# Liz490/multimodal_alzheimer

Measured on AMD Instinct MI355X. Metric: volumes/sec fwd+bwd, 3D-ResNet-10 @128^3 bf16, 1/2/4/8 MI355X; % HBM roofline, higher is better.
Workload: dtype bf16; 1 GPU; BASELINE config 2: Anat_CNN ResNet-10 MRI-only, 1x128^3, batch 8/GPU, weighted CE, Adam, fwd+bwd+step; global_batch=8, parallelism=dp1, step_launch=hip graph replay

## Files before the change

multimodal_alzheimer_amd/csrc/common.h:

```cpp
#pragma once
#include <hip/hip_runtime.h>
#include <stdint.h>

#include "../../include/mmad.h"

typedef float f32x4 __attribute__((ext_vector_type(4)));
typedef __bf16 bf16x8 __attribute__((ext_vector_type(8)));
typedef __bf16 bf16x4 __attribute__((ext_vector_type(4)));
typedef unsigned short u16;
typedef unsigned short u16x8 __attribute__((ext_vector_type(8)));
typedef unsigned short u16x4 __attribute__((ext_vector_type(4)));
typedef uint32_t u32x4 __attribute__((ext_vector_type(4)));

#define LDS_AS __attribute__((address_space(3)))

template <int N>
__device__ __forceinline__ void wait_vm_lgkm0() {
  static_assert(N >= 0 && N <= 63, "vmcnt immediate (6 bits)");
  asm volatile("s_waitcnt vmcnt(%0) lgkmcnt(0)" ::"i"(N) : "memory");
}

__device__ __forceinline__ void raw_barrier() {
  __builtin_amdgcn_s_barrier();
  asm volatile("" ::: "memory");
}

__device__ __forceinline__ void glds16_asm(const void* gsrc, uint32_t lds_addr) {
  uint32_t keep;
  asm volatile(
      "s_mov_b32 %0, m0\n\ts_mov_b32 m0, %2\n\ts_nop 0\n\t"
      "global_load_lds_dwordx4 %1, off\n\ts_mov_b32 m0, %0"
      : "=&s"(keep)
      : "v"(gsrc), "s"(lds_addr)
      : "memory");
}
__device__ __forceinline__ void buf_lds16_asm(uint32_t voff, __amdgpu_buffer_rsrc_t rsrc,
                                              uint32_t lds_addr) {
  uint32_t keep;
  asm volatile(
      "s_mov_b32 %0, m0\n\ts_mov_b32 m0, %3\n\ts_nop 0\n\t"
      "buffer_load_dwordx4 %1, %2, 0 offen lds\n\ts_mov_b32 m0, %0"
      : "=&s"(keep)
      : "v"(voff), "s"(rsrc), "s"(lds_addr)
      : "memory");
}
__device__ __forceinline__ uint32_t lds_addr_of(const void* p) {
  return __builtin_amdgcn_readfirstlane((uint32_t)(uintptr_t)(const LDS_AS void*)p);
}

__device__ __forceinline__ float bf2f(u16 v) { return __uint_as_float(((uint32_t)v) << 16); }
typedef float f32x2 __attribute__((ext_vector_type(2)));
typedef __bf16 bf16x2 __attribute__((ext_vector_type(2)));
__device__ __forceinline__ uint32_t pack_bf16x2(float a, float b) {
  return __builtin_bit_cast(uint32_t, __builtin_convertvector((f32x2){a, b}, bf16x2));
}
__device__ __forceinline__ u16 f2bf(float f) { return (u16)(pack_bf16x2(f, 0.f) & 0xffffu); }

template <typename T> struct Elt;
template <> struct Elt<float> {
  static __device__ __forceinline__ float ld(const float* p, int64_t i) { return p[i]; }
  static __device__ __forceinline__ void st(float* p, int64_t i, float v) { p[i] = v; }
  static constexpr int VEC = 4;
};
template <> struct Elt<u16> {
  static __device__ __forceinline__ float ld(const u16* p, int64_t i) { return bf2f(p[i]); }
  static __device__ __forceinline__ void st(u16* p, int64_t i, float v) { p[i] = f2bf(v); }
  static constexpr int VEC = 8;
};

template <typename T> struct Chunk;
template <> struct Chunk<float> {
  static constexpr int N = 4;
  static __device__ __forceinline__ void load(const float* p, float* v) {
    f32x4 c = *reinterpret_cast<const f32x4*>(p);
    v[0] = c[0]; v[1] = c[1]; v[2] = c[2]; v[3] = c[3];
  }
  static __device__ __forceinline__ void store(float* p, const float* v) {
    f32x4 c; c[0] = v[0]; c[1] = v[1]; c[2] = v[2]; c[3] = v[3];
    *reinterpret_cast<f32x4*>(p) = c;
  }
};
template <> struct Chunk<u16> {
  static constexpr int N = 8;
  static __device__ __forceinline__ void load(const u16* p, float* v) {
    u16x8 c = *reinterpret_cast<const u16x8*>(p);
#pragma unroll
    for (int i = 0; i < 8; ++i) v[i] = bf2f(c[i]);
  }
  static __device__ __forceinline__ void store(u16* p, const float* v) {
    u32x4 c;
#pragma unroll
    for (int i = 0; i < 4; ++i) c[i] = pack_bf16x2(v[2 * i], v[2 * i + 1]);
    *reinterpret_cast<u32x4*>(p) = c;
  }
};

__device__ __forceinline__ u32x4 epi_res_relu(u32x4 v, const u16* res, int relu) {
  float f[8];
  Chunk<u16>::load(reinterpret_cast<const u16*>(&v), f);
  if (res != nullptr) {
    float r[8];
    Chunk<u16>::load(res, r);
#pragma unroll
    for (int e = 0; e < 8; ++e) f[e] += r[e];
  }
  if (relu) {
#pragma unroll
    for (int e = 0; e < 8; ++e) f[e] = fmaxf(f[e], 0.f);
  }
  u32x4 o;
  Chunk<u16>::store(reinterpret_cast<u16*>(&o), f);
  return o;
}

__device__ __forceinline__ float bn_affine(float y, float scale, float shift) {
  return __builtin_fmaf(y, scale, shift);
}
template <typename T>
__device__ __forceinline__ float as_stored(float v) {
  if constexpr (sizeof(T) == 2) return bf2f(f2bf(v));
  else return v;
}

__device__ __forceinline__ float wave_sum(float v) {
#pragma unroll
  for (int o = 32; o > 0; o >>= 1) v += __shfl_xor(v, o, 64);
  return v;
}
__device__ __forceinline__ double wave_sum_d(double v) {
#pragma unroll
  for (int o = 32; o > 0; o >>= 1) v += __shfl_xor(v, o, 64);
  return v;
}

__device__ __forceinline__ uint64_t mix64(uint64_t z) {
  z += 0x9E3779B97F4A7C15ull;
  z = (z ^ (z >> 30)) * 0xBF58476D1CE4E5B9ull;
  z = (z ^ (z >> 27)) * 0x94D049BB133111EBull;
  return z ^ (z >> 31);
}

static inline int hip_status(hipError_t e) { return e == hipSuccess ? MMAD_OK : MMAD_EHIP + (int)e; }
static inline int launch_status() { return hip_status(hipGetLastError()); }
static inline hipStream_t as_stream(void* s) { return reinterpret_cast<hipStream_t>(s); }
static inline int64_t cdiv(int64_t a, int64_t b) { return (a + b - 1) / b; }

__global__ void zero_fill_kernel(uint32_t* __restrict__ p, int64_t words);
int zero_fill(void* p, int64_t bytes, hipStream_t st);
static inline bool is_pow2(int64_t v) { return v > 0 && (v & (v - 1)) == 0; }
static inline int ilog2(int64_t v) { int r = 0; while ((int64_t(1) << r) < v) ++r; return r; }
```

multimodal_alzheimer_amd/csrc/lattice8.hip:

```cpp
#include <atomic>
#include <cstdlib>
#include <type_traits>

#include "bnsum.h"
#include "common.h"
#include "patchconv.h"

namespace {

constexpr int S8 = 8;
constexpr int NC = 8;
constexpr int PL8 = S8 * S8 * NC;
constexpr int RB8 = 64;
constexpr int KC8 = RB8 / 2;
constexpr int PLANE8 = PL8 * RB8;
constexpr int BN8 = 64;
constexpr int BTAP8 = BN8 * RB8;
constexpr int TPS8 = 9;
constexpr int BSLOT8 = TPS8 * BTAP8;
constexpr int NSL8 = 2;
constexpr int NPL8 = 2;
constexpr int RING8 = NPL8 * PLANE8;
constexpr int ZERO8 = RING8 + NSL8 * BSLOT8;
constexpr int MAIN8 = ZERO8 + RB8;
constexpr int CROW8 = BN8 * 2 + 16;
constexpr int EPI8 = PL8 * CROW8 + 7 * 2 * BN8 * 4;
constexpr int LDS8 = MAIN8 > EPI8 ? MAIN8 : EPI8;
constexpr int NT8 = 512;

struct L8 {
  int nb, Cs, Nd, Kpad, nbn, nchunk;
  const u16* res;
  int relu;
  int D, H, W, nz;
  const u16* bny;
  const float *bnsc, *bnsh, *bnmu, *bnis;
  float* bnparts;
};

__device__ __forceinline__ int swz8(int row) { return 3 * ((row >> 3) & 1); }

template <int TN, int NFR>
struct Fr8 {
  bf16x8 b[TN];
  bf16x8 a[NFR];
};

template <int WM, int KY, int WR>
__device__ constexpr bool row_ok(int f) {
  return WR * WM + (f >> 2) + KY >= 0 && WR * WM + (f >> 2) + KY < S8;
}

template <int TN, int WM, int KY, int KX, int WR>
__device__ __forceinline__ void read8(const char* bsl, const char* pl, const uint32_t (&ao)[2],
                                      const char* zp, bool lhi, Fr8<TN, 4 * WR>& f) {
#pragma unroll
  for (int j = 0; j < TN; ++j)
    f.b[j] = *reinterpret_cast<const bf16x8*>(bsl + (KX + 1) * BTAP8 + j * 16 * RB8);
#pragma unroll
  for (int q = 0; q < 4 * WR; ++q) {
    if (row_ok<WM, KY, WR>(q)) {
      constexpr int dummy = 0;
      const int ty = WR * WM + (q >> 2) + KY + dummy, x0 = 2 * (q & 3) + KX;
      const int base = (ty * S8 + x0) * NC * RB8;
      const char* p = pl + base + ao[KX & 1];
      if (KX == -1 && (q & 3) == 0) p = lhi ? p : zp;
      if (KX == 1 && (q & 3) == 3) p = lhi ? zp : p;
      f.a[q] = *reinterpret_cast<const bf16x8*>(p);
    }
  }
}

template <int TN, int WM, int KY, int WR>
__device__ __forceinline__ void mma8(f32x4 (&acc)[4 * WR][TN], const Fr8<TN, 4 * WR>& f) {
#pragma unroll
  for (int q = 0; q < 4 * WR; ++q)
    if (row_ok<WM, KY, WR>(q)) {
#pragma unroll
      for (int j = 0; j < TN; ++j)
        acc[q][j] = __builtin_amdgcn_mfma_f32_16x16x32_bf16(f.a[q], f.b[j], acc[q][j], 0, 0, 0);
    }
}

template <int TN, int WM, int KY, int WR>
__device__ __forceinline__ void stage8(f32x4 (&acc)[4 * WR][TN], const char* bsl,
                                       const char* pl, const uint32_t (&ao)[2], const char* zp,
                                       bool lhi) {
  Fr8<TN, 4 * WR> f0, f1;
  read8<TN, WM, KY, -1, WR>(bsl, pl, ao, zp, lhi, f0);
  read8<TN, WM, KY, 0, WR>(bsl, pl, ao, zp, lhi, f1);
  mma8<TN, WM, KY, WR>(acc, f0);
  read8<TN, WM, KY, 1, WR>(bsl, pl, ao, zp, lhi, f0);
  mma8<TN, WM, KY, WR>(acc, f1);
  mma8<TN, WM, KY, WR>(acc, f0);
}

template <int TN, bool RAG, int WR>
__global__ __launch_bounds__(NT8) void lattice8_conv_kernel(L8 g, const u16* __restrict__ src,
                                                            const u16* __restrict__ wgt,
                                                            const float* __restrict__ bias,
                                                            u16* __restrict__ dst,
                                                            float* __restrict__ stats) {
  extern __shared__ __attribute__((aligned(16))) char smem[];
  char* ring = smem + RING8;
  const int tid = threadIdx.x, lane = tid & 63;
  const int wave = __builtin_amdgcn_readfirstlane(tid >> 6);
  const int nwg = gridDim.x, bid = blockIdx.x;
  const int xcd = bid & 7, qq = nwg >> 3, rr = nwg & 7;
  const int tile = (xcd < rr ? xcd * (qq + 1) : rr * (qq + 1) + (xcd - rr) * qq) + (bid >> 3);
  const int nt = tile % g.nbn;
  const int t2 = tile / g.nbn;
  const int NZ = RAG ? g.nz : S8;
  const int tz = t2 % NZ, n = t2 / NZ;
  constexpr int NFR = 4 * WR;
  constexpr int NWM = 8 / WR, NWN = WR;
  constexpr int BW = 16 * TN * NWN;
  const int n0 = nt * BW;
  constexpr int E = 2 * S8;

  if (tid < RB8 / 16)
    *reinterpret_cast<u32x4*>(smem + ZERO8 + tid * 16) = u32x4{0u, 0u, 0u, 0u};

  const int lrow = lane >> 2;
  int rzk[4];
  uint32_t pofs[4];
#pragma unroll
  for (int k = 0; k < 4; ++k) {
    const int row = (wave * 4 + k) * 16 + lrow;
    const int pos = row >> 3, c = row & 7;
    const int ty = pos >> 3, tx = pos & 7;
    const int pch = (lane & 3) ^ swz8(row);
    if constexpr (RAG) {
      const int y = ((c >> 1) & 1) + 2 * ty, x = (c & 1) + 2 * tx;
      pofs[k] = (uint32_t)((((c >> 2) * g.H + y) * g.W + x) * g.Cs + pch * 8) * 2u;
      rzk[k] = (y < g.H && x < g.W) ? (c >> 2) : -(1 << 20);
    } else {
      const int v = ((c >> 2) * E + ((c >> 1) & 1) + 2 * ty) * E + (c & 1) + 2 * tx;
      pofs[k] = (uint32_t)(v * g.Cs + pch * 8) * 2u;
      rzk[k] = 0;
    }
  }
  const int64_t svox = RAG ? (int64_t)g.D * g.H * g.W : (int64_t)E * E * E;
  const __amdgpu_buffer_rsrc_t rsx = __builtin_amdgcn_make_buffer_rsrc(
      (void*)(src + (int64_t)n * svox * g.Cs), 0,
      (int)__builtin_amdgcn_readfirstlane((uint32_t)(svox * g.Cs * 2)), 0x00020000);
  auto issue_plane_at = [&](int p, int zr, int cc) {
    char* pb = smem + p * PLANE8;
    if constexpr (RAG) {
      constexpr uint32_t OOB = 0x80000000u;
      const int zp = 2 * (tz - 1 + zr);
      const uint32_t zoff = (uint32_t)(zp * g.H * g.W * g.Cs + cc * KC8) * 2u;
#pragma unroll
      for (int k = 0; k < 4; ++k) {
        const bool ok = rzk[k] >= 0 && rzk[k] + zp >= 0 && rzk[k] + zp < g.D;
        buf_lds16_asm(ok ? pofs[k] + zoff : OOB, rsx, lds_addr_of(pb + (wave * 4 + k) * 1024));
      }
    } else {
      const uint32_t zoff = (uint32_t)(2 * (tz - 1 + zr) * E * E * g.Cs + cc * KC8) * 2u;
#pragma unroll
      for (int k = 0; k < 4; ++k) {
        uint32_t o = pofs[k];
        asm volatile("" : "+v"(o));
        buf_lds16_asm(o + zoff, rsx, lds_addr_of(pb + (wave * 4 + k) * 1024));
      }
    }
  };
  constexpr int QB = BW / 16;
  constexpr int NQ9 = 9 * BW / 16, WI9 = (NQ9 + 7) / 8;
  const __amdgpu_buffer_rsrc_t rsw = __builtin_amdgcn_make_buffer_rsrc(
      (void*)wgt, 0, (int)__builtin_amdgcn_readfirstlane((uint32_t)(g.Nd * g.Kpad * 2)),
      0x00020000);
  uint32_t wofs9[WI9];
#pragma unroll
  for (int h = 0; h < WI9; ++h) {
    const int q = min(wave + 8 * h, NQ9 - 1);
    const int row = (q % QB) * 16 + lrow;
    wofs9[h] = (uint32_t)((n0 + row) * g.Kpad + ((lane & 3) ^ swz8(row)) * 8 + (q / QB) * g.Cs) *
               2u;
  }
  auto issue_b9 = [&](int cc, int t0, int sl) {
    const uint32_t so = (uint32_t)(t0 * g.Cs + cc * KC8) * 2u;
#pragma unroll
    for (int h = 0; h < WI9; ++h) {
      const int q = min(wave + 8 * h, NQ9 - 1);
      uint32_t o = wofs9[h];
      asm volatile("" : "+v"(o));
      buf_lds16_asm(o + so, rsw, lds_addr_of(ring + sl * BSLOT8 + (q / QB) * BTAP8 + (q % QB) * 1024));
    }
  };
  const int kz0 = tz == 0 ? 0 : -1, kz1 = tz == NZ - 1 ? 0 : 1;
  const int nkz = kz1 - kz0 + 1;
  const int wm = wave % NWM, wn = wave / NWM;
  const int lr = lane & 15, lk = lane >> 4;
  const bool lhi = (lr >> 3) != 0;
  uint32_t ao[2];
  ao[0] = lr * RB8 + ((lk ^ swz8(lr)) << 4);
  ao[1] = lr * RB8 + ((lk ^ (3 - swz8(lr))) << 4);
  const char* zp = smem + ZERO8 + (lk << 4);
  const uint32_t b_lane = (wn * 16 * TN + lr) * RB8 + ((lk ^ swz8(lr)) << 4);
  f32x4 acc[NFR][TN];
#pragma unroll
  for (int i = 0; i < NFR; ++i)
#pragma unroll
    for (int j = 0; j < TN; ++j) acc[i][j] = f32x4{0.f, 0.f, 0.f, 0.f};

  auto run9 = [&](auto wmc) {
    constexpr int WM = decltype(wmc)::value;
    const int n9 = g.nchunk * nkz;
    issue_plane_at(0, kz0 + 1, 0);
    issue_b9(0, (kz0 + 1) * 9, 0);
    int e = 0;
    for (int c = 0; c < g.nchunk; ++c)
      for (int kzi = 0; kzi < nkz; ++kzi, ++e) {
        wait_vm_lgkm0<0>();
        raw_barrier();
        if (e + 1 < n9) {
          const int c1 = kzi + 1 < nkz ? c : c + 1, kz1 = kz0 + (kzi + 1 < nkz ? kzi + 1 : 0);
          issue_plane_at((e + 1) & 1, kz1 + 1, c1);
          issue_b9(c1, (kz1 + 1) * 9, (e + 1) & 1);
        }
        const char* pl = smem + (e & 1) * PLANE8;
        const char* bs = ring + (e & 1) * BSLOT8 + b_lane;
        stage8<TN, WM, -1, WR>(acc, bs, pl, ao, zp, lhi);
        stage8<TN, WM, 0, WR>(acc, bs + 3 * BTAP8, pl, ao, zp, lhi);
        stage8<TN, WM, 1, WR>(acc, bs + 6 * BTAP8, pl, ao, zp, lhi);
      }
  };
  auto dispatch = [&](auto wmc) {
    if constexpr (decltype(wmc)::value < NWM) run9(wmc);
  };
  switch (wm) {
    case 0: dispatch(std::integral_constant<int, 0>{}); break;
    case 1: dispatch(std::integral_constant<int, 1>{}); break;
    case 2: dispatch(std::integral_constant<int, 2>{}); break;
    case 3: dispatch(std::integral_constant<int, 3>{}); break;
    case 4: dispatch(std::integral_constant<int, 4>{}); break;
    case 5: dispatch(std::integral_constant<int, 5>{}); break;
    case 6: dispatch(std::integral_constant<int, 6>{}); break;
    default: dispatch(std::integral_constant<int, 7>{}); break;
  }
  __syncthreads();

  auto dst_vox = [&](int row) -> int64_t {
    const int pos = row >> 3, c = row & 7;
    const int ty = pos >> 3, tx = pos & 7;
    if constexpr (RAG) {
      const int z = (c >> 2) + 2 * tz, y = ((c >> 1) & 1) + 2 * ty, x = (c & 1) + 2 * tx;
      if (z >= g.D || y >= g.H || x >= g.W) return -1;
      return (((int64_t)n * g.D + z) * g.H + y) * g.W + x;
    }
    return (((int64_t)n * E + (c >> 2) + 2 * tz) * E + ((c >> 1) & 1) + 2 * ty) * E + (c & 1) +
           2 * tx;
  };
  u16* ctile = reinterpret_cast<u16*>(smem);
  uint32_t vmask = 0xffffffffu;
  if constexpr (RAG) {
    vmask = 0;
#pragma unroll 1
    for (int b = 0; b < 4 * NFR; ++b) {
      const int q = b >> 2, e = b & 3;
      const int row = ((WR * wm + (q >> 2)) * S8 + 2 * (q & 3)) * NC + lk * 4 + e;
      if (dst_vox(row) >= 0) vmask |= 1u << b;
    }
  }
  float cs[TN], cq[TN];
#pragma unroll
  for (int j = 0; j < TN; ++j) {
    cs[j] = 0.f;
    cq[j] = 0.f;
    const int col = wn * 16 * TN + j * 16 + lr;
    const float bv = bias != nullptr ? bias[n0 + col] : 0.f;
#pragma unroll
    for (int q = 0; q < NFR; ++q) {
      const int ty = WR * wm + (q >> 2);
#pragma unroll
      for (int e = 0; e < 4; ++e) {
        const int row = (ty * S8 + 2 * (q & 3)) * NC + lk * 4 + e;
        const float v = acc[q][j][e] + bv;
        ctile[row * (CROW8 / 2) + col] = f2bf(v);
        if ((vmask >> (q * 4 + e)) & 1u) {
          cs[j] += v;
          cq[j] += v * v;
        }
      }
    }
  }
  __syncthreads();
  constexpr int CPR = BW / 8;
  static_assert(NT8 % CPR == 0, "a thread keeps one channel vector in the store loop");
  if (g.bny != nullptr) {
    BnSum bs;
    bs.init(g.bnsc, g.bnsh, g.bnmu, g.bnis, n0 + (tid % CPR) * 8);
#pragma unroll
    for (int hh = 0; hh < PL8 * CPR / NT8; ++hh) {
      const int qd = tid + NT8 * hh;
      const int row = qd / CPR, c8 = qd % CPR;
      const int64_t dv = dst_vox(row);
      if (RAG && dv < 0) continue;
      const int64_t o = dv * g.Nd + n0 + c8 * 8;
      const u32x4 v = *reinterpret_cast<const u32x4*>(reinterpret_cast<const char*>(ctile) +
                                                      row * CROW8 + c8 * 16);
      const u32x4 yv = *reinterpret_cast<const u32x4*>(g.bny + o);
      *reinterpret_cast<u32x4*>(dst + o) = v;
      bs.add(v, yv);
    }
    __syncthreads();
    bnsum_flush(bs, reinterpret_cast<float*>(smem), CPR, NT8, g.bnparts, n * NZ + tz, g.Nd, n0);
    return;
  }
#pragma unroll
  for (int hh = 0; hh < PL8 * CPR / NT8; ++hh) {
    const int qd = tid + NT8 * hh;
    const int row = qd / CPR, c8 = qd % CPR;
    const int64_t dv = dst_vox(row);
    if (RAG && dv < 0) continue;
    const int64_t o = dv * g.Nd + n0 + c8 * 8;
    u32x4 v = *reinterpret_cast<const u32x4*>(reinterpret_cast<const char*>(ctile) +
                                              row * CROW8 + c8 * 16);
    if (g.res != nullptr || g.relu) v = epi_res_relu(v, g.res ? g.res + o : nullptr, g.relu);
    *reinterpret_cast<u32x4*>(dst + o) = v;
  }
  if (stats != nullptr) {
    float* red = reinterpret_cast<float*>(smem + PL8 * CROW8);
#pragma unroll
    for (int j = 0; j < TN; ++j) {
      cs[j] += __shfl_xor(cs[j], 16, 64);
      cs[j] += __shfl_xor(cs[j], 32, 64);
      cq[j] += __shfl_xor(cq[j], 16, 64);
      cq[j] += __shfl_xor(cq[j], 32, 64);
    }
    if (wm > 0 && lk == 0) {
#pragma unroll
      for (int j = 0; j < TN; ++j) {
        const int col = wn * 16 * TN + j * 16 + lr;
        red[(wm - 1) * 2 * BW + col] = cs[j];
        red[(wm - 1) * 2 * BW + BW + col] = cq[j];
      }
    }
    __syncthreads();
    if (wm == 0 && lk == 0) {
      const int mt = n * NZ + tz;
#pragma unroll
      for (int j = 0; j < TN; ++j) {
        const int col = wn * 16 * TN + j * 16 + lr;
        float ss = cs[j], qs = cq[j];
        for (int w = 1; w < NWM; ++w) {
          ss += red[(w - 1) * 2 * BW + col];
          qs += red[(w - 1) * 2 * BW + BW + col];
        }
        stats[((int64_t)mt * 2) * g.Nd + n0 + col] = ss;
        stats[((int64_t)mt * 2 + 1) * g.Nd + n0 + col] = qs;
      }
    }
  }
}

std::atomic<int> g_lattice8_mode{-1};
int lattice8_mode() {
  int v = g_lattice8_mode.load(std::memory_order_relaxed);
  if (v < 0) {
    const char* e = getenv("MMAD_LATTICE8");
    int expect = -1;
    g_lattice8_mode.compare_exchange_strong(expect, e ? atoi(e) : 1);
    v = g_lattice8_mode.load(std::memory_order_relaxed);
  }
  return v;
}

int l8_rows() {
  static const int v = [] {
    const char* e = getenv("MMAD_L8_ROWS");
    return e && atoi(e) == 2 ? 2 : 1;
  }();
  return v;
}

}

namespace mmad_lattice8 {

int set_mode(int v) {
  const int prev = lattice8_mode();
  if (v >= 0) g_lattice8_mode.store(v, std::memory_order_relaxed);
  return prev;
}

static bool exact8(const mmad_patch::Geo& q) {
  constexpr int E = 2 * S8;
  return q.Ds == E && q.Hs == E && q.Ws == E && q.Dd == E && q.Hd == E && q.Wd == E;
}
static bool ragged8(const mmad_patch::Geo& q) {
  static const int mode = [] {
    const char* e = getenv("MMAD_LATTICE_RAGGED");
    return e ? atoi(e) : 1;
  }();
  return mode > 0 && !exact8(q) && q.Ds == q.Dd && q.Hs == q.Hd && q.Ws == q.Wd &&
         (q.Hs + 1) / 2 <= S8 && (q.Ws + 1) / 2 <= S8 &&
         (int64_t)q.Ds * q.Hs * q.Ws * q.Cs * 2 < (int64_t(1) << 31);
}
static int planes8(const mmad_patch::Geo& q) { return exact8(q) ? S8 : (q.Ds + 1) / 2; }

bool ok(const mmad_patch::Geo& q) {
  if (lattice8_mode() <= 0) return false;
  if (q.KD != 3 || q.KH != 3 || q.KW != 3) return false;
  if (q.dd != 2 || q.dh != 2 || q.dw != 2 || q.pd != 2 || q.ph != 2 || q.pw != 2) return false;
  if (!exact8(q) && !ragged8(q)) return false;
  if (q.Cs % KC8 || q.Nd % 32 || q.Kpad != 27 * q.Cs) return false;
  if (lattice8_mode() == 1 && (int64_t)q.nb * planes8(q) * (q.Nd / 32) < 256) return false;
  return (int64_t)q.Ds * q.Hs * q.Ws * q.Cs * 2 < (int64_t(1) << 31) &&
         (int64_t)q.Nd * q.Kpad * 2 < (int64_t(1) << 31);
}

int64_t tiles(const mmad_patch::Geo& q) { return (int64_t)q.nb * planes8(q); }

int fwd(const mmad_patch::Geo& q, const void* src, const void* wp, const float* bias,
        void* dst, float* stats, void* stream) {
  if (!mmad_lattice8::ok(q)) return MMAD_EUNSUPPORTED;
  auto attr1 = [](const void* k) {
    return hipFuncSetAttribute(k, hipFuncAttributeMaxDynamicSharedMemorySize, LDS8) ==
           hipSuccess;
  };
  static const bool attr =
      attr1((const void*)lattice8_conv_kernel<2, false, 2>) &&
      attr1((const void*)lattice8_conv_kernel<1, false, 2>) &&
      attr1((const void*)lattice8_conv_kernel<2, true, 2>) &&
      attr1((const void*)lattice8_conv_kernel<1, true, 2>) &&
      attr1((const void*)lattice8_conv_kernel<4, false, 1>) &&
      attr1((const void*)lattice8_conv_kernel<2, false, 1>) &&
      attr1((const void*)lattice8_conv_kernel<4, true, 1>) &&
      attr1((const void*)lattice8_conv_kernel<2, true, 1>);
  if (!attr) return MMAD_EUNSUPPORTED;
  const bool rag = !exact8(q);
  const int nz = planes8(q);
  const bool wide = q.Nd % BN8 == 0 && (int64_t)q.nb * nz * (q.Nd / BN8) >= 256;
  L8 g{};
  g.nb = q.nb; g.Cs = q.Cs; g.Nd = q.Nd; g.Kpad = q.Kpad;
  g.nbn = q.Nd / (wide ? BN8 : 32);
  g.nchunk = q.Cs / KC8;
  g.res = reinterpret_cast<const u16*>(q.res);
  g.relu = q.relu;
  g.D = q.Ds; g.H = q.Hs; g.W = q.Ws; g.nz = nz;
  g.bny = reinterpret_cast<const u16*>(q.bny);
  g.bnsc = q.bnsc; g.bnsh = q.bnsh; g.bnmu = q.bnmu; g.bnis = q.bnis;
  g.bnparts = q.bnparts;
  if (g.bny != nullptr && (stats != nullptr || g.res != nullptr || g.relu || bias != nullptr))
    return MMAD_EUNSUPPORTED;
  const int64_t nblk = (int64_t)q.nb * nz * g.nbn;
  auto go = [&](auto kern) {
    hipLaunchKernelGGL(kern, dim3((unsigned)nblk), dim3(NT8), LDS8, as_stream(stream), g,
                       (const u16*)src, (const u16*)wp, bias, (u16*)dst, stats);
  };
  if (l8_rows() == 1) {
    if (wide) rag ? go(lattice8_conv_kernel<4, true, 1>) : go(lattice8_conv_kernel<4, false, 1>);
    else rag ? go(lattice8_conv_kernel<2, true, 1>) : go(lattice8_conv_kernel<2, false, 1>);
  } else {
    if (wide) rag ? go(lattice8_conv_kernel<2, true, 2>) : go(lattice8_conv_kernel<2, false, 2>);
    else rag ? go(lattice8_conv_kernel<1, true, 2>) : go(lattice8_conv_kernel<1, false, 2>);
  }
  return launch_status();
}

}
```

multimodal_alzheimer_amd/csrc/pwgrad.hip:

```cpp
#include "common.h"
#include "patchconv.h"

namespace {

constexpr int PW_KC = 32;
constexpr int PW_TY = 8;
constexpr int PW_XW = 32;
constexpr int PW_YR = PW_TY + 2;
constexpr int PW_XSLOTS = 4;
constexpr int PW_YROW = 128;
constexpr int PW_YST = 2 * PW_XW * PW_YROW;
constexpr int PW_YSLOTS = 4;
constexpr int PW_NTHR = 512;
constexpr uint32_t PW_OOB = 0x80000000u;
template <int MODE>
struct PWC {
  static constexpr bool LAT = MODE == 1, W16 = MODE == 2, W40 = MODE == 3;
  static constexpr int XR = LAT ? 40 : W16 ? 18 : W40 ? 50 : PW_XW + 2;
  static constexpr int SPP = W40 ? 5 : 4;
  static constexpr int YRI = W16 ? 18 : PW_YR;
  static constexpr int XROWS = YRI * XR;
  static constexpr int XDMA = (XROWS + 15) / 16;
  static constexpr int XSLOT = XDMA * 1024;
  static constexpr int Y_OFF = PW_XSLOTS * XSLOT;
  static constexpr int LDS = Y_OFF + PW_YSLOTS * PW_YST;
  static constexpr int NXMAX = (XDMA + 7) / 8;
};

struct PWG {
  int nb, Cs, Nd, D, H, K;
  int zr;
  int ng;
};

__device__ __forceinline__ int pw_wsz128(int r) { return 2 * ((r >> 1) & 1) + 4 * ((r >> 3) & 1); }

template <int MODE>
__global__ __launch_bounds__(PW_NTHR) void pwgrad_kernel(PWG g, const u16* __restrict__ x,
                                                         const u16* __restrict__ dy,
                                                         float* __restrict__ ws) {
  using C = PWC<MODE>;
  constexpr bool LAT = C::LAT, W16 = C::W16, W40 = C::W40;
  constexpr int XR = C::XR, SPP = C::SPP;
  extern __shared__ __attribute__((aligned(16))) char smem[];
  const int tid = threadIdx.x, lane = tid & 63;
  const int wave = __builtin_amdgcn_readfirstlane(tid >> 6);
  const int nci = g.Cs / PW_KC, nco = g.Nd / 64;
  const int nwg = gridDim.x, bid = blockIdx.x;
  const int xcd = bid & 7, qq = nwg >> 3, rr = nwg & 7;
  const int tile = (xcd < rr ? xcd * (qq + 1) : rr * (qq + 1) + (xcd - rr) * qq) + (bid >> 3);
  const int cot = tile % nco, t2 = tile / nco;
  const int cit = t2 % nci, split = t2 / nci;
  const int nyt = LAT ? 2 / g.ng : W16 ? 1 : g.H / PW_TY, nzr = (LAT ? 8 : g.D) / g.zr;
  const int zi = split % nzr, yt = (split / nzr) % nyt, n = split / (nzr * nyt);
  const int rz = LAT ? yt : 0;
  const int co0 = cot * 64, ci0 = cit * PW_KC, y0 = LAT || W16 ? 0 : yt * PW_TY, z0 = zi * g.zr;
  constexpr int VW = LAT || W16 ? 16 : W40 ? 40 : PW_XW;

  const int64_t vox = LAT ? (int64_t)16 * 16 * 16 : (int64_t)g.D * g.H * VW;
  const __amdgpu_buffer_rsrc_t rsx = __builtin_amdgcn_make_buffer_rsrc(
      (void*)(x + n * vox * g.Cs), 0, (int)__builtin_amdgcn_readfirstlane((int)(vox * g.Cs * 2)),
      0x00020000);
  const __amdgpu_buffer_rsrc_t rsy = __builtin_amdgcn_make_buffer_rsrc(
      (void*)(dy + n * vox * g.Nd), 0, (int)__builtin_amdgcn_readfirstlane((int)(vox * g.Nd * 2)),
      0x00020000);
  const uint32_t smem_l = lds_addr_of(smem);

  const int nx = wave + 8 * (C::NXMAX - 1) < C::XDMA ? C::NXMAX : C::NXMAX - 1;
  auto xoff = [&](int h) -> uint32_t {
    const int q = wave + 8 * h, row = 16 * q + (lane >> 2);
    if constexpr (LAT) {
      const int yv = row / XR - 1, ps = row % XR, sg = ps / 10, xv = ps % 10 - 1;
      const bool ok = row < C::XROWS && (unsigned)yv < 8u && (unsigned)xv < 8u;
      const int vy = (sg >> 1) + 2 * yv, vx = (sg & 1) + 2 * xv;
      return ok ? (uint32_t)(((vy * 16 + vx) * g.Cs + ci0 + (lane & 3) * 8) * 2) : PW_OOB;
    } else if constexpr (W16) {
      const int yv = row / XR - 1, xv = row % XR - 1;
      const bool ok = row < C::XROWS && (unsigned)yv < (unsigned)g.H && (unsigned)xv < 16u;
      return ok ? (uint32_t)(((yv * 16 + xv) * g.Cs + ci0 + (lane & 3) * 8) * 2) : PW_OOB;
    } else if constexpr (W40) {
      const int yv = y0 - 1 + row / XR, ps = row % XR, xv = 8 * (ps / 10) + ps % 10 - 1;
      const bool ok = row < C::XROWS && (unsigned)yv < (unsigned)g.H && (unsigned)xv < 40u;
      return ok ? (uint32_t)(((yv * 40 + xv) * g.Cs + ci0 + (lane & 3) * 8) * 2) : PW_OOB;
    } else {
      const int yv = y0 - 1 + row / XR, xv = row % XR - 1;
      const bool ok = row < C::XROWS && (unsigned)yv < (unsigned)g.H &&
                      (unsigned)xv < (unsigned)PW_XW;
      return ok ? (uint32_t)(((yv * PW_XW + xv) * g.Cs + ci0 + (lane & 3) * 8) * 2) : PW_OOB;
    }
  };
  const uint32_t xplane = LAT ? (uint32_t)(16 * 16 * g.Cs * 2) : (uint32_t)(g.H * VW * g.Cs * 2);
  const int gstride = g.zr + 2;
  auto issue_x = [&](int e, int rz) {
    const uint32_t slot = smem_l + (uint32_t)(((unsigned)e % PW_XSLOTS) * C::XSLOT);
    if (LAT && e >= gstride) {
      e -= gstride;
      rz += 1;
    }
    const int zp = z0 - 1 + e;
    const bool zin = !LAT || (unsigned)zp < 8u;
    const uint32_t pz = LAT ? (uint32_t)(rz + 2 * zp) * xplane : (uint32_t)zp * xplane;
#pragma unroll
    for (int h = 0; h < C::NXMAX; ++h)
      if (h < nx)
        buf_lds16_asm(zin ? xoff(h) + pz : PW_OOB, rsx, slot + (uint32_t)((wave + 8 * h) * 1024));
  };
  const int yr = wave * 8 + (lane >> 3);
  const int yvox = LAT ? ((((yr >> 3) & 3) >> 1) + 2 * (yr >> 5)) * 16 + (((yr >> 3) & 3) & 1) +
                             2 * (yr & 7)
                       : yr;
  const uint32_t ylane = (uint32_t)(((W40 ? (lane >> 3) : yvox) * g.Nd + co0 +
                                     ((lane & 7) ^ pw_wsz128(yr)) * 8) * 2);
  auto issue_y = [&](int o, int m, int sl, int rz) {
    uint32_t base;
    if constexpr (W40) {
      const int j = 4 * (2 * m + (wave >> 2)) + (wave & 3);
      base = (uint32_t)((((z0 + o) * g.H + y0 + j / 5) * 40 + 8 * (j % 5)) * g.Nd * 2);
    } else {
      base = LAT ? (uint32_t)(((rz + 2 * (z0 + o)) * 16 + 4 * m) * 16) * (uint32_t)g.Nd * 2
             : W16 ? (uint32_t)(((z0 + o) * g.H + 4 * m) * 16) * (uint32_t)g.Nd * 2
                   : (uint32_t)(((z0 + o) * g.H + y0 + 2 * m) * PW_XW) * (uint32_t)g.Nd * 2;
    }
    buf_lds16_asm(base + ylane, rsy, smem_l + (uint32_t)(C::Y_OFF + sl * PW_YST + wave * 1024));
  };

  const int cf = wave & 1, tg = wave >> 1;
  const int t0 = tg * 7, nt = tg == 3 ? 6 : 7;
  const int lk = lane >> 4, q4 = (lane & 15) >> 2, p4 = lane & 3;
  const int rsel = 8 * lk + q4;
  uint32_t ya_lo[4], ya_hi[4];
#pragma unroll
  for (int i = 0; i < 4; ++i) {
    const int col = i * 16 + 4 * p4;
    ya_lo[i] = (uint32_t)(rsel * PW_YROW + (((col >> 3) ^ pw_wsz128(rsel)) << 4) + (col & 7) * 2);
    ya_hi[i] = (uint32_t)((rsel + 4) * PW_YROW + (((col >> 3) ^ pw_wsz128(rsel + 4)) << 4) +
                          (col & 7) * 2);
  }
  const uint32_t xb = (uint32_t)((LAT ? 10 * lk + q4 : W16 ? 18 * (lk >> 1) + 8 * (lk & 1) + q4
                                  : W40 ? q4 : rsel) *
                                     64 + cf * 32 + 8 * p4);
  uint32_t xk[W40 ? 5 : 1];
#pragma unroll
  for (int kt = 0; kt < (W40 ? 5 : 1); ++kt) {
    const int j = 4 * kt + lk;
    xk[kt] = W40 ? (uint32_t)(((j / 5) * XR + (j % 5) * 10) * 64) : 0u;
  }
  f32x4 acc[4][7];
#pragma unroll
  for (int i = 0; i < 4; ++i)
#pragma unroll
    for (int k = 0; k < 7; ++k) acc[i][k] = f32x4{0.f, 0.f, 0.f, 0.f};

  auto tr8 = [](const char* p) {
    return __builtin_amdgcn_ds_read_tr16_b64_v4bf16((LDS_AS bf16x4*)p);
  };
  auto prologue = [&](int rz) {
    issue_x(0, rz);
    issue_x(1, rz);
    issue_x(2, rz);
    issue_y(0, 0, 0, rz);
    issue_y(0, 1, 1, rz);
  };
  prologue(rz);
  const int ng = LAT ? g.ng : 1;
  const int nstage = ng * g.zr * SPP;

  struct PFr { bf16x8 a[4], b[7]; };
  auto run = [&](auto tgc) {
    constexpr int TG = decltype(tgc)::value;
    constexpr int NT = TG == 3 ? 6 : 7;
    const char* xbase[3];
    auto y_on = [](int t, int yl) constexpr {
      return !LAT || ((unsigned)(yl + (t / 3) % 3 - 1) < 8u);
    };
    auto kread = [&](const char* yimg, auto qc, auto ylc, PFr& f) {
      constexpr int Q = decltype(qc)::value, YL = decltype(ylc)::value;
#pragma unroll
      for (int i = 0; i < 4; ++i)
        f.a[i] = __builtin_shufflevector(tr8(yimg + Q * PW_XW * PW_YROW + ya_lo[i]),
                                         tr8(yimg + Q * PW_XW * PW_YROW + ya_hi[i]), 0, 1, 2, 3,
                                         4, 5, 6, 7);
      auto one = [&](auto kc) {
        constexpr int K = decltype(kc)::value;
        if constexpr (K < NT && y_on(TG * 7 + K, YL)) {
          constexpr int t = TG * 7 + K;
          constexpr int kz = t / 9, ky = (t / 3) % 3, kx = t % 3;
          const char* img;
          if constexpr (W40) {
            constexpr int r0 = ((YL / 5) * 4 + ky) * XR + kx;
            img = xbase[kz] + xk[YL % 5] + r0 * 64;
          } else {
            constexpr int r0 = ((W16 ? 2 : 1) * YL + ky) * XR + kx;
            img = xbase[kz] + r0 * 64;
          }
          f.b[K] = __builtin_shufflevector(tr8(img), tr8(img + 4 * 64), 0, 1, 2, 3, 4, 5, 6, 7);
        }
      };
      one(std::integral_constant<int, 0>{});
      one(std::integral_constant<int, 1>{});
      one(std::integral_constant<int, 2>{});
      one(std::integral_constant<int, 3>{});
      one(std::integral_constant<int, 4>{});
      one(std::integral_constant<int, 5>{});
      one(std::integral_constant<int, 6>{});
    };
    auto kmma = [&](const PFr& f, auto ylc) {
      constexpr int YL = decltype(ylc)::value;
      auto one = [&](auto kc) {
        constexpr int K = decltype(kc)::value;
        if constexpr (K < NT && y_on(TG * 7 + K, YL)) {
#pragma unroll
          for (int i = 0; i < 4; ++i)
            acc[i][K] = __builtin_amdgcn_mfma_f32_16x16x32_bf16(f.a[i], f.b[K], acc[i][K], 0, 0,
                                                                0);
        }
      };
      one(std::integral_constant<int, 0>{});
      one(std::integral_constant<int, 1>{});
      one(std::integral_constant<int, 2>{});
      one(std::integral_constant<int, 3>{});
      one(std::integral_constant<int, 4>{});
      one(std::integral_constant<int, 5>{});
      one(std::integral_constant<int, 6>{});
    };
#pragma unroll 1
    for (int o = 0; o < ng * g.zr; ++o) {
      const bool second = o >= g.zr;
      const int v = o + (second ? 2 : 0);
      if (LAT && o == g.zr) {
        raw_barrier();
        issue_x(v + 1, rz);
        issue_x(v + 2, rz);
      }
#pragma unroll
      for (int j = 0; j < 3; ++j) {
        uint32_t b = (uint32_t)(((unsigned)(v + j) % PW_XSLOTS) * C::XSLOT) + xb;
        asm volatile("v_mov_b32 %0, %1" : "=v"(b) : "v"(b));
        xbase[j] = smem + b;
      }
      const bool xnext = v + 3 < ng * gstride;
      auto stage = [&](auto mc) {
        constexpr int M = decltype(mc)::value;
        const int s = o * SPP + M;
        if (s + 1 >= nstage || (LAT && M == 0 && o == g.zr)) {
          wait_vm_lgkm0<0>();
        } else if ((M == 1 || M == 2) && xnext) {
          if (nx == 4) wait_vm_lgkm0<5>();
          else if (nx == 3) wait_vm_lgkm0<4>();
          else wait_vm_lgkm0<3>();
        } else {
          wait_vm_lgkm0<1>();
        }
        raw_barrier();
        if (s + 2 < nstage) {
          const int p2 = (int)((unsigned)(s + 2) / SPP), g2 = p2 >= g.zr ? 1 : 0;
          issue_y(p2 - g2 * g.zr, (int)((unsigned)(s + 2) % SPP), (int)((unsigned)(s + 2) % PW_YSLOTS), rz + g2);
        }
        if (M == 0 && xnext) issue_x(v + 3, rz);
        int yoff = C::Y_OFF + (int)((unsigned)s % PW_YSLOTS) * PW_YST;
        asm volatile("" : "+s"(yoff));
        const char* yimg = smem + yoff;
        PFr f0, f1;
        kread(yimg, std::integral_constant<int, 0>{}, std::integral_constant<int, 2 * M>{}, f0);
        kread(yimg, std::integral_constant<int, 1>{}, std::integral_constant<int, 2 * M + 1>{},
              f1);
        kmma(f0, std::integral_constant<int, 2 * M>{});
        kmma(f1, std::integral_constant<int, 2 * M + 1>{});
      };
      stage(std::integral_constant<int, 0>{});
      stage(std::integral_constant<int, 1>{});
      stage(std::integral_constant<int, 2>{});
      stage(std::integral_constant<int, 3>{});
      if constexpr (SPP == 5) stage(std::integral_constant<int, 4>{});
    }
  };
  switch (tg) {
    case 0: run(std::integral_constant<int, 0>{}); break;
    case 1: run(std::integral_constant<int, 1>{}); break;
    case 2: run(std::integral_constant<int, 2>{}); break;
    default: run(std::integral_constant<int, 3>{}); break;
  }

  float* out = ws + (int64_t)split * g.Nd * g.K;
  const int lr = lane & 15;
#pragma unroll
  for (int k = 0; k < 7; ++k) {
    if (k < nt) {
      const int kcol = (t0 + k) * g.Cs + ci0 + cf * 16 + lr;
#pragma unroll
      for (int i = 0; i < 4; ++i)
#pragma unroll
        for (int r = 0; r < 4; ++r)
          out[(int64_t)(co0 + i * 16 + lk * 4 + r) * g.K + kcol] = acc[i][k][r];
    }
  }
}

bool pw_on() {
  static const bool v = [] {
    const char* e = getenv("MMAD_PWGRAD");
    return e == nullptr || atoi(e) != 0;
  }();
  return v;
}
bool lat_on() {
  static const bool v = [] {
    const char* e = getenv("MMAD_PWGRAD_LAT");
    return e == nullptr || atoi(e) != 0;
  }();
  return v;
}

bool w16_on() {
  static const bool v = [] {
    const char* e = getenv("MMAD_PWGRAD_W16");
    return e == nullptr || atoi(e) != 0;
  }();
  return v;
}
bool w16_geo(const mmad_patch::Geo& q) {
  return q.KD == 3 && q.KH == 3 && q.KW == 3 && q.dd == 1 && q.dh == 1 && q.dw == 1 &&
         q.pd == 1 && q.ph == 1 && q.pw == 1 && q.Ds == q.Dd && q.Hs == q.Hd && q.Ws == q.Wd &&
         q.Wd == 16 && q.Hd == 16 && q.Dd >= 4;
}
bool w40_on() {
  static const bool v = [] {
    const char* e = getenv("MMAD_PWGRAD_W40");
    return e == nullptr || atoi(e) != 0;
  }();
  return v;
}
bool w40_geo(const mmad_patch::Geo& q) {
  return q.KD == 3 && q.KH == 3 && q.KW == 3 && q.dd == 1 && q.dh == 1 && q.dw == 1 &&
         q.pd == 1 && q.ph == 1 && q.pw == 1 && q.Ds == q.Dd && q.Hs == q.Hd && q.Ws == q.Wd &&
         q.Wd == 40 && q.Hd % PW_TY == 0 && q.Dd >= 4;
}
bool lat_geo(const mmad_patch::Geo& q) {
  return q.KD == 3 && q.KH == 3 && q.KW == 3 && q.dd == 2 && q.dh == 2 && q.dw == 2 &&
         q.pd == 2 && q.ph == 2 && q.pw == 2 && q.Ds == 16 && q.Hs == 16 && q.Ws == 16 &&
         q.Dd == 16 && q.Hd == 16 && q.Wd == 16;
}

int lat_ng(const mmad_patch::Geo& q) {
  static const int force1 = [] {
    const char* e = getenv("MMAD_PWGRAD_LAT_NG");
    return e != nullptr && atoi(e) == 1;
  }();
  if (!lat_geo(q) || force1) return 1;
  return (int64_t)q.nb * (q.Cs / PW_KC) * (q.Nd / 64) >= 256 ? 2 : 1;
}

int pw_zr(const mmad_patch::Geo& q) {
  if (lat_geo(q)) {
    const int64_t base = (int64_t)q.nb * (2 / lat_ng(q)) * (q.Cs / PW_KC) * (q.Nd / 64);
    int zr = 8;
    while (zr > 2 && base * (8 / zr) < 256) zr /= 2;
    return zr;
  }
  const int64_t base =
      (int64_t)q.nb * (w16_geo(q) ? 1 : q.Hd / PW_TY) * (q.Cs / PW_KC) * (q.Nd / 64);
  int zr = q.Dd;
  while (zr > 4 && zr % 2 == 0 && base * (q.Dd / zr) < 256) zr /= 2;
  return zr;
}

}

namespace mmad_pwgrad {

bool ok(const mmad_patch::Geo& q) {
  if (!pw_on()) return false;
  if (q.Cs % PW_KC || q.Nd % 64 || q.Kpad != 27 * q.Cs) return false;
  if (lat_geo(q)) return lat_on() && (int64_t)4096 * std::max(q.Cs, q.Nd) * 2 < (int64_t(1) << 30);
  if (w16_geo(q)) {
    if (!w16_on() || (int64_t)q.Dd * 256 * std::max(q.Cs, q.Nd) * 2 >= (int64_t(1) << 30))
      return false;
    const int zr = pw_zr(q);
    return q.Dd % zr == 0 && zr >= 2;
  }
  if (w40_geo(q)) {
    if (!w40_on() || (int64_t)q.Dd * q.Hd * 40 * std::max(q.Cs, q.Nd) * 2 >= (int64_t(1) << 30))
      return false;
    const int zr = pw_zr(q);
    return q.Dd % zr == 0 && zr >= 2;
  }
  if (q.KD != 3 || q.KH != 3 || q.KW != 3 || q.dd != 1 || q.dh != 1 || q.dw != 1) return false;
  if (q.pd != 1 || q.ph != 1 || q.pw != 1) return false;
  if (q.Ds != q.Dd || q.Hs != q.Hd || q.Ws != q.Wd || q.Wd != PW_XW) return false;
  if (q.Hd % PW_TY || q.Dd < 4) return false;
  if ((int64_t)q.Dd * q.Hd * PW_XW * std::max(q.Cs, q.Nd) * 2 >= (int64_t(1) << 30)) return false;
  const int zr = pw_zr(q);
  return q.Dd % zr == 0 && zr >= 2;
}

int64_t splits(const mmad_patch::Geo& q) {
  if (lat_geo(q)) return (int64_t)q.nb * (2 / lat_ng(q)) * (8 / pw_zr(q));
  if (w16_geo(q)) return (int64_t)q.nb * (q.Dd / pw_zr(q));
  return (int64_t)q.nb * (q.Hd / PW_TY) * (q.Dd / pw_zr(q));
}

int64_t workspace(const mmad_patch::Geo& q) {
  return mmad_pwgrad::splits(q) * q.Nd * 27 * q.Cs * 4;
}

int wgrad(const mmad_patch::Geo& q, const void* x, const void* dy, float* ws, int* nsplit,
          void* stream) {
  if (!mmad_pwgrad::ok(q)) return MMAD_EUNSUPPORTED;
  static const bool attr =
      hipFuncSetAttribute((const void*)pwgrad_kernel<0>,
                          hipFuncAttributeMaxDynamicSharedMemorySize, PWC<0>::LDS) == hipSuccess &&
      hipFuncSetAttribute((const void*)pwgrad_kernel<1>,
                          hipFuncAttributeMaxDynamicSharedMemorySize, PWC<1>::LDS) == hipSuccess &&
      hipFuncSetAttribute((const void*)pwgrad_kernel<2>,
                          hipFuncAttributeMaxDynamicSharedMemorySize, PWC<2>::LDS) == hipSuccess &&
      hipFuncSetAttribute((const void*)pwgrad_kernel<3>,
                          hipFuncAttributeMaxDynamicSharedMemorySize, PWC<3>::LDS) == hipSuccess;
  if (!attr) return MMAD_EUNSUPPORTED;
  const int mode = lat_geo(q) ? 1 : w16_geo(q) ? 2 : w40_geo(q) ? 3 : 0;
  PWG g{};
  g.nb = q.nb; g.Cs = q.Cs; g.Nd = q.Nd; g.D = q.Dd; g.H = q.Hd; g.K = 27 * q.Cs;
  g.zr = pw_zr(q);
  g.ng = lat_ng(q);
  const int64_t sp = mmad_pwgrad::splits(q);
  const int64_t nblk = sp * (q.Cs / PW_KC) * (q.Nd / 64);
  if (mode == 1)
    hipLaunchKernelGGL(pwgrad_kernel<1>, dim3((unsigned)nblk), dim3(PW_NTHR), PWC<1>::LDS,
                       as_stream(stream), g, (const u16*)x, (const u16*)dy, ws);
  else if (mode == 2)
    hipLaunchKernelGGL(pwgrad_kernel<2>, dim3((unsigned)nblk), dim3(PW_NTHR), PWC<2>::LDS,
                       as_stream(stream), g, (const u16*)x, (const u16*)dy, ws);
  else if (mode == 3)
    hipLaunchKernelGGL(pwgrad_kernel<3>, dim3((unsigned)nblk), dim3(PW_NTHR), PWC<3>::LDS,
                       as_stream(stream), g, (const u16*)x, (const u16*)dy, ws);
  else
    hipLaunchKernelGGL(pwgrad_kernel<0>, dim3((unsigned)nblk), dim3(PW_NTHR), PWC<0>::LDS,
                       as_stream(stream), g, (const u16*)x, (const u16*)dy, ws);
  *nsplit = (int)sp;
  return launch_status();
}

}
```

Before: 2775 volumes/sec.

## Interleave LDS DMA issues between MMA stages and batch buffer loads under one m0 setup

In the lattice8 conv kernel, the next plane and weight-slot prefetches now issue between the three MMA stages instead of right after the barrier. They are emitted as grouped buffer_load...lds sequences that share one m0 save/restore and a scalar offset. A predicate zeroes the buffer range so the final iteration's DMA becomes a no-op rather than a branch, and the kernel drains with a trailing waitcnt. Tile indices and offsets are made wave-uniform through readfirstlane. In pwgrad's lattice mode, the X-tile issue moves between the two MMAs. The aim is to overlap global-to-LDS traffic with matrix work and cut issue overhead, at the cost of extra no-op loads and scheduling barriers that restrict compiler freedom.

```diff
diff --git a/multimodal_alzheimer_amd/csrc/common.h b/multimodal_alzheimer_amd/csrc/common.h
--- a/multimodal_alzheimer_amd/csrc/common.h
+++ b/multimodal_alzheimer_amd/csrc/common.h
@@ -44,6 +44,40 @@
       : "v"(voff), "s"(rsrc), "s"(lds_addr)
       : "memory");
 }
+#define MMAD_DMA1(i)                                                                      \
+  "s_add_u32 m0, %[l" #i "], %[add]\n\ts_nop 0\n\t"                                       \
+  "buffer_load_dwordx4 %[v" #i "], %[rs], %[so] offen lds\n\t"
+#define MMAD_DMA_OPS(i) [v##i] "v"(voff[i]), [l##i] "s"(lds[i])
+template <int N>
+__device__ __forceinline__ void buf_lds16_group_asm(const uint32_t (&voff)[N],
+                                                    __amdgpu_buffer_rsrc_t rsrc, uint32_t soff,
+                                                    const uint32_t (&lds)[N], uint32_t lds_add) {
+  static_assert(N >= 3 && N <= 5, "group sizes in use");
+  uint32_t keep;
+  if constexpr (N == 3)
+    asm volatile("s_mov_b32 %[k], m0\n\t" MMAD_DMA1(0) MMAD_DMA1(1) MMAD_DMA1(2)
+                 "s_mov_b32 m0, %[k]"
+                 : [k] "=&s"(keep)
+                 : [rs] "s"(rsrc), [so] "s"(soff), [add] "s"(lds_add), MMAD_DMA_OPS(0),
+                   MMAD_DMA_OPS(1), MMAD_DMA_OPS(2)
+                 : "memory", "scc");
+  else if constexpr (N == 4)
+    asm volatile("s_mov_b32 %[k], m0\n\t" MMAD_DMA1(0) MMAD_DMA1(1) MMAD_DMA1(2) MMAD_DMA1(3)
+                 "s_mov_b32 m0, %[k]"
+                 : [k] "=&s"(keep)
+                 : [rs] "s"(rsrc), [so] "s"(soff), [add] "s"(lds_add), MMAD_DMA_OPS(0),
+                   MMAD_DMA_OPS(1), MMAD_DMA_OPS(2), MMAD_DMA_OPS(3)
+                 : "memory", "scc");
+  else
+    asm volatile("s_mov_b32 %[k], m0\n\t" MMAD_DMA1(0) MMAD_DMA1(1) MMAD_DMA1(2) MMAD_DMA1(3)
+                     MMAD_DMA1(4) "s_mov_b32 m0, %[k]"
+                 : [k] "=&s"(keep)
+                 : [rs] "s"(rsrc), [so] "s"(soff), [add] "s"(lds_add), MMAD_DMA_OPS(0),
+                   MMAD_DMA_OPS(1), MMAD_DMA_OPS(2), MMAD_DMA_OPS(3), MMAD_DMA_OPS(4)
+                 : "memory", "scc");
+}
+#undef MMAD_DMA_OPS
+#undef MMAD_DMA1
 __device__ __forceinline__ uint32_t lds_addr_of(const void* p) {
   return __builtin_amdgcn_readfirstlane((uint32_t)(uintptr_t)(const LDS_AS void*)p);
 }
diff --git a/multimodal_alzheimer_amd/csrc/lattice8.hip b/multimodal_alzheimer_amd/csrc/lattice8.hip
--- a/multimodal_alzheimer_amd/csrc/lattice8.hip
+++ b/multimodal_alzheimer_amd/csrc/lattice8.hip
@@ -108,10 +108,11 @@
   const int nwg = gridDim.x, bid = blockIdx.x;
   const int xcd = bid & 7, qq = nwg >> 3, rr = nwg & 7;
   const int tile = (xcd < rr ? xcd * (qq + 1) : rr * (qq + 1) + (xcd - rr) * qq) + (bid >> 3);
-  const int nt = tile % g.nbn;
+  const int nt = __builtin_amdgcn_readfirstlane(tile % g.nbn);
   const int t2 = tile / g.nbn;
   const int NZ = RAG ? g.nz : S8;
-  const int tz = t2 % NZ, n = t2 / NZ;
+  const int tz = __builtin_amdgcn_readfirstlane(t2 % NZ);
+  const int n = __builtin_amdgcn_readfirstlane(t2 / NZ);
   constexpr int NFR = 4 * WR;
   constexpr int NWM = 8 / WR, NWN = WR;
   constexpr int BW = 16 * TN * NWN;
@@ -141,52 +142,50 @@
     }
   }
   const int64_t svox = RAG ? (int64_t)g.D * g.H * g.W : (int64_t)E * E * E;
-  const __amdgpu_buffer_rsrc_t rsx = __builtin_amdgcn_make_buffer_rsrc(
-      (void*)(src + (int64_t)n * svox * g.Cs), 0,
-      (int)__builtin_amdgcn_readfirstlane((uint32_t)(svox * g.Cs * 2)), 0x00020000);
-  auto issue_plane_at = [&](int p, int zr, int cc) {
-    char* pb = smem + p * PLANE8;
+  const u16* sbase = src + (int64_t)n * svox * g.Cs;
+  const uint32_t xbytes = __builtin_amdgcn_readfirstlane((uint32_t)(svox * g.Cs * 2));
+  const uint32_t smem_l = lds_addr_of(smem);
+  uint32_t pdst[4];
+#pragma unroll
+  for (int k = 0; k < 4; ++k) pdst[k] = smem_l + (uint32_t)((wave * 4 + k) * 1024);
+  auto issue_plane_at = [&](int p, int zr, int cc, bool live) {
+    const __amdgpu_buffer_rsrc_t rsx =
+        __builtin_amdgcn_make_buffer_rsrc((void*)sbase, 0, (int)(live ? xbytes : 0u), 0x00020000);
     if constexpr (RAG) {
       constexpr uint32_t OOB = 0x80000000u;
       const int zp = 2 * (tz - 1 + zr);
-      const uint32_t zoff = (uint32_t)(zp * g.H * g.W * g.Cs + cc * KC8) * 2u;
+      const uint32_t zoff = __builtin_amdgcn_readfirstlane(
+          (uint32_t)(zp * g.H * g.W * g.Cs + cc * KC8) * 2u);
+      uint32_t vo[4];
 #pragma unroll
       for (int k = 0; k < 4; ++k) {
         const bool ok = rzk[k] >= 0 && rzk[k] + zp >= 0 && rzk[k] + zp < g.D;
-        buf_lds16_asm(ok ? pofs[k] + zoff : OOB, rsx, lds_addr_of(pb + (wave * 4 + k) * 1024));
+        vo[k] = ok ? pofs[k] : OOB;
       }
+      buf_lds16_group_asm(vo, rsx, zoff, pdst, (uint32_t)(p * PLANE8));
     } else {
-      const uint32_t zoff = (uint32_t)(2 * (tz - 1 + zr) * E * E * g.Cs + cc * KC8) * 2u;
-#pragma unroll
-      for (int k = 0; k < 4; ++k) {
-        uint32_t o = pofs[k];
-        asm volatile("" : "+v"(o));
-        buf_lds16_asm(o + zoff, rsx, lds_addr_of(pb + (wave * 4 + k) * 1024));
-      }
+      const uint32_t zoff = __builtin_amdgcn_readfirstlane(
+          (uint32_t)(2 * (tz - 1 + zr) * E * E * g.Cs + cc * KC8) * 2u);
+      buf_lds16_group_asm(pofs, rsx, zoff, pdst, (uint32_t)(p * PLANE8));
     }
   };
   constexpr int QB = BW / 16;
   constexpr int NQ9 = 9 * BW / 16, WI9 = (NQ9 + 7) / 8;
-  const __amdgpu_buffer_rsrc_t rsw = __builtin_amdgcn_make_buffer_rsrc(
-      (void*)wgt, 0, (int)__builtin_amdgcn_readfirstlane((uint32_t)(g.Nd * g.Kpad * 2)),
-      0x00020000);
-  uint32_t wofs9[WI9];
+  const uint32_t wbytes = __builtin_amdgcn_readfirstlane((uint32_t)(g.Nd * g.Kpad * 2));
+  uint32_t wofs9[WI9], wdst[WI9];
 #pragma unroll
   for (int h = 0; h < WI9; ++h) {
     const int q = min(wave + 8 * h, NQ9 - 1);
     const int row = (q % QB) * 16 + lrow;
     wofs9[h] = (uint32_t)((n0 + row) * g.Kpad + ((lane & 3) ^ swz8(row)) * 8 + (q / QB) * g.Cs) *
                2u;
-  }
-  auto issue_b9 = [&](int cc, int t0, int sl) {
-    const uint32_t so = (uint32_t)(t0 * g.Cs + cc * KC8) * 2u;
-#pragma unroll
-    for (int h = 0; h < WI9; ++h) {
-      const int q = min(wave + 8 * h, NQ9 - 1);
-      uint32_t o = wofs9[h];
-      asm volatile("" : "+v"(o));
-      buf_lds16_asm(o + so, rsw, lds_addr_of(ring + sl * BSLOT8 + (q / QB) * BTAP8 + (q % QB) * 1024));
-    }
+    wdst[h] = smem_l + (uint32_t)(RING8 + (q / QB) * BTAP8 + (q % QB) * 1024);
+  }
+  auto issue_b9 = [&](int cc, int t0, int sl, bool live) {
+    const __amdgpu_buffer_rsrc_t rsw =
+        __builtin_amdgcn_make_buffer_rsrc((void*)wgt, 0, (int)(live ? wbytes : 0u), 0x00020000);
+    const uint32_t so = __builtin_amdgcn_readfirstlane((uint32_t)(t0 * g.Cs + cc * KC8) * 2u);
+    buf_lds16_group_asm(wofs9, rsw, so, wdst, (uint32_t)(sl * BSLOT8));
   };
   const int kz0 = tz == 0 ? 0 : -1, kz1 = tz == NZ - 1 ? 0 : 1;
   const int nkz = kz1 - kz0 + 1;
@@ -207,24 +206,29 @@
   auto run9 = [&](auto wmc) {
     constexpr int WM = decltype(wmc)::value;
     const int n9 = g.nchunk * nkz;
-    issue_plane_at(0, kz0 + 1, 0);
-    issue_b9(0, (kz0 + 1) * 9, 0);
+    issue_plane_at(0, kz0 + 1, 0, true);
+    issue_b9(0, (kz0 + 1) * 9, 0, true);
     int e = 0;
     for (int c = 0; c < g.nchunk; ++c)
       for (int kzi = 0; kzi < nkz; ++kzi, ++e) {
         wait_vm_lgkm0<0>();
         raw_barrier();
-        if (e + 1 < n9) {
-          const int c1 = kzi + 1 < nkz ? c : c + 1, kz1 = kz0 + (kzi + 1 < nkz ? kzi + 1 : 0);
-          issue_plane_at((e + 1) & 1, kz1 + 1, c1);
-          issue_b9(c1, (kz1 + 1) * 9, (e + 1) & 1);
-        }
+        const bool more = e + 1 < n9;
+        const int c1 = kzi + 1 < nkz ? c : c + 1, kz1 = kz0 + (kzi + 1 < nkz ? kzi + 1 : 0);
+        const int s1 = (e + 1) & 1;
         const char* pl = smem + (e & 1) * PLANE8;
         const char* bs = ring + (e & 1) * BSLOT8 + b_lane;
         stage8<TN, WM, -1, WR>(acc, bs, pl, ao, zp, lhi);
+        __builtin_amdgcn_sched_barrier(0);
+        issue_plane_at(s1, kz1 + 1, c1, more);
+        __builtin_amdgcn_sched_barrier(0);
         stage8<TN, WM, 0, WR>(acc, bs + 3 * BTAP8, pl, ao, zp, lhi);
+        __builtin_amdgcn_sched_barrier(0);
+        issue_b9(c1, (kz1 + 1) * 9, s1, more);
+        __builtin_amdgcn_sched_barrier(0);
         stage8<TN, WM, 1, WR>(acc, bs + 6 * BTAP8, pl, ao, zp, lhi);
       }
+    wait_vm_lgkm0<0>();
   };
   auto dispatch = [&](auto wmc) {
     if constexpr (decltype(wmc)::value < NWM) run9(wmc);
diff --git a/multimodal_alzheimer_amd/csrc/pwgrad.hip b/multimodal_alzheimer_amd/csrc/pwgrad.hip
--- a/multimodal_alzheimer_amd/csrc/pwgrad.hip
+++ b/multimodal_alzheimer_amd/csrc/pwgrad.hip
@@ -256,7 +256,8 @@
           const int p2 = (int)((unsigned)(s + 2) / SPP), g2 = p2 >= g.zr ? 1 : 0;
           issue_y(p2 - g2 * g.zr, (int)((unsigned)(s + 2) % SPP), (int)((unsigned)(s + 2) % PW_YSLOTS), rz + g2);
         }
-        if (M == 0 && xnext) issue_x(v + 3, rz);
+        constexpr bool XLATE = LAT;
+        if (!XLATE && M == 0 && xnext) issue_x(v + 3, rz);
         int yoff = C::Y_OFF + (int)((unsigned)s % PW_YSLOTS) * PW_YST;
         asm volatile("" : "+s"(yoff));
         const char* yimg = smem + yoff;
@@ -265,6 +266,11 @@
         kread(yimg, std::integral_constant<int, 1>{}, std::integral_constant<int, 2 * M + 1>{},
               f1);
         kmma(f0, std::integral_constant<int, 2 * M>{});
+        if (XLATE && M == 0 && xnext) {
+          __builtin_amdgcn_sched_barrier(0);
+          issue_x(v + 3, rz);
+          __builtin_amdgcn_sched_barrier(0);
+        }
         kmma(f1, std::integral_constant<int, 2 * M + 1>{});
       };
       stage(std::integral_constant<int, 0>{});
```

Measured after the change: 2795 volumes/sec, median of 6. About the same (+0.7%).
